# igashov/DiffLinker

Hardware: AMD Instinct MI355X
Metric: molecules/sec (500-step sample_chain) (higher is better)
Workload: dtype f32 (f16x3 split MFMA, fp32 accumulate)

## Files before the change

### difflinker_amd/csrc/egnn_fc.hip

```cpp
#include <hip/hip_runtime.h>
#include <stdint.h>
#include <stdlib.h>
#include <string.h>
#include <math.h>
#include <cmath>

#include <algorithm>
#include <atomic>
#include <vector>

#include "../../include/difflinker_hip.h"
#include "pack_layout.h"


namespace {

constexpr int LDH = 132;
constexpr int NMAX = 55;
constexpr int NQMAX = 2 * NMAX;
constexpr int THREADS = 512;
constexpr int NWAVES = THREADS / 64;
constexpr int GWAVES = 8;
constexpr int GTHREADS = 64 * GWAVES;
constexpr int L_A = 0;
// ... 18 lines not shown
constexpr int L_ZROW = L_XS + 4 * 56;
static_assert(L_ZROW + HID <= L_X0 && 56 >= NMAX + 1 && (L_ZROW % 4) == 0, "the zero row sits in the team-only part of the coordinate rows");
constexpr size_t LDS_BYTES = size_t(L_TOTAL) * 4;
static_assert(LDS_BYTES <= 163840, "LDS layout exceeds 160 KiB");
static_assert((L_B % 4) == 0 && (L_C % 4) == 0 && (L_W % 4) == 0 && (L_VEC % 4) == 0 && (L_XS % 4) == 0 &&
              (L_X0 % 4) == 0 && (L_Z % 4) == 0 && (L_DUMMY % 4) == 0, "16-byte alignment");
constexpr int L_TRIP3 = L_A + 2 * ST_CHUNK;
constexpr int L_AGGX3 = L_TRIP3 + 4 * 256;
static_assert(L_AGGX3 + 4 * (NMAX + 1) <= L_W && (L_TRIP3 % 4) == 0, "version-3 coordinate scratch must fit the h region behind the ring");

constexpr int TM_EPOCH = 2;
constexpr int TM_FAIL = 3;
constexpr int TM_ROWS = 4;
constexpr int TM_FLAGS = 6;
constexpr int TM_S = 8, TM_RANK = 9, TM_NOWN = 10;
constexpr int MS_NRCV = 12;
constexpr int MS_FULL = 13;
constexpr int CX_V3 = 38;

struct Lds {
    float *A, *B, *C, *W, *vec, *xs, *x0, *aggx, *z, *lm, *frag;
    int *idx, *rcv, *rpos, *misc;
    unsigned* fmax;
    float* dummy;
    int w;
};

__device__ __forceinline__ Lds lds_view(float* base) {
    Lds v;
    v.w = __builtin_amdgcn_readfirstlane(int(threadIdx.x) >> 6);
// ... 1232 lines not shown
    const float4* s4 = reinterpret_cast<const float4*>(wimg) + lane;
#pragma unroll
    for (int it = 0; it < ST_PIECES; ++it) {
        const int piece = HALF * 32 + it * 4 + hw;
        __builtin_amdgcn_global_load_lds((gptr_t)(s4 + piece * 64), (lptr_t)(v.W + piece * 256), 16, 0, 0);
    }
}
template <int N>
__device__ __forceinline__ void st_wait_vm() {
    if constexpr (N <= 0) asm volatile("s_waitcnt vmcnt(0)" ::: "memory");
    else asm volatile("s_waitcnt vmcnt(%0)" :: "n"(N) : "memory");
}
template <int V>
struct IC { static constexpr int value = V; };

template <bool TEAM, bool POST, bool NEXT_EQ>
__device__ __forceinline__ void stream_phase(const Lds& v, Prof& pf, const AggRegs* ar) {
    constexpr int NC = (POST ? 6 : 0) + 4;
    constexpr int C_P = POST ? 6 : 0;
    const PassCtx cx = pass_ctx(v);
    const LaneIds q = lane_ids(v);
    const int tid = q.tid, w = q.w, lane = q.lane;
    const int nb = cx.nb;
    const int nown = TEAM ? ctx_i(v, TM_NOWN) : nb;
    float* hs = cx.hs;
    const int pass_open = cx.pass + 1;
    const float* wp = ctx_p<const float>(v, CX_WP);
    const int sub = ctx_i(v, CX_SUB);
    const float* g = POST ? cx.g : nullptr;
    const float* nxb = pass_weights(wp, pass_open, sub);
    const NextPass nx = {nxb, NEXT_EQ};
    const float* sc = POST ? g + G_SCALE : nullptr;
    const float* scn = nxb + (NEXT_EQ ? E_SCALE : G_SCALE);
    const float* vecn = nxb + (NEXT_EQ ? E_VEC : G_VEC);
    float* lds0 = v.A - L_A;
    const bool loader = w >= ST_AWAVES;
    const int hw = w - ST_AWAVES, wa = w;
    const int n = lane & 15, kg = lane >> 4;
    const int ta = wa;
// ... 14 lines not shown
    float hmax = 0.f, aggmax = 0.f, s_agg = 1.f, s_t = 1.f, s_hn = 1.f, inv2 = 1.f;
    if constexpr (POST) {
        hmax = __uint_as_float(v.fmax[FM_H0 + par]);
        aggmax = __uint_as_float(v.fmax[FM_AGG]);
        s_agg = scale_for(aggmax);
        const float y3b = cload(sc, SC_L1_W3A) * hmax + cload(sc, SC_L1_W3B) * aggmax + cload(sc, SC_B3);
        s_t = scale_for(y3b);
        const float hnb = hmax + cload(sc, SC_L1_W4) * y3b + cload(sc, SC_B4);
        s_hn = scale_for(hnb);
        if (tid == 0 && (beyond_f16_range(aggmax) || beyond_f16_range(y3b) || beyond_f16_range(hnb))) atomicOr(&v.misc[1], NAN_RANGE | 3);
        inv2 = inv_pow2(s_t * cload(sc, 4));
    }
    const float s_h0 = scale_for(__uint_as_float(v.fmax[FM_H0 + par]));
    const float s_hf = POST ? s_hn : s_h0;
    constexpr int AGG_OFF = st_slot_off(st_slot(3, NC));
    if constexpr (POST) {
#pragma unroll
        for (int k = 0; k < 4; ++k) {
            const int e = tid + THREADS * k;
            if (e < nown * 32) *reinterpret_cast<float4*>(lds0 + AGG_OFF + (e >> 5) * LDH + 4 * (e & 31)) = ar->v[k];
        }
    }
    if (loader) {
        st_issue<st_slot(0, NC)>(lds0, chunk_src(0), hw, lane);
        prof_event(pf, w, lane, 200);
        auto lstep = [&](auto C_) {
            constexpr int C = decltype(C_)::value;
            constexpr int behind = (C >= 1 && C + 1 < NC ? ST_PIECES : 0) + (C == NC - 2 ? ST_PIECES : 0) + (C == NC - 1 ? 2 * ST_PIECES : 0);
            st_wait_vm<behind>();
            fine_event(pf, w, lane, 220 + C);
            lds_barrier();
// ... 10 lines not shown
        lstep(IC<0>{}); lstep(IC<1>{}); lstep(IC<2>{}); lstep(IC<3>{});
        if constexpr (NC > 4) { lstep(IC<4>{}); lstep(IC<5>{}); }
        if constexpr (NC > 6) { lstep(IC<6>{}); lstep(IC<7>{}); }
        if constexpr (NC > 8) { lstep(IC<8>{}); lstep(IC<9>{}); }
        fine_event(pf, w, lane, 240);
        lds_barrier();
        prof_event(pf, w, lane, 250);
    } else {
    BOp bh, bagg, bout, bin;
    floatx4 acc[4];
    float4 t0p[4];
    float4 res2[8], bb4[8];
    float4 Pout[8], Qout[8];
    float hm = 0.f;
    float S1 = 1.f;
    if (!TEAM) {
        const float x2 = __uint_as_float(v.fmax[FM_X2]), x02 = __uint_as_float(v.fmax[FM_X02]);
        S1 = fminf(scale_for(4.0f * x2) * scale_for(cload(scn, 6)), scale_for(4.0f * x02) * scale_for(cload(scn, 7)));
    }
    const float live = valid ? 1.0f : 0.0f;
    if (awave) {
        const float sb = s_h0 * live;
#pragma unroll
        for (int sl = 0; sl < 4; ++sl) {
            const float4 a = hold[2 * sl], c4 = hold[2 * sl + 1];
            const float u[8] = {a.x * sb, a.y * sb, a.z * sb, a.w * sb, c4.x * sb, c4.y * sb, c4.z * sb, c4.w * sb};
            split8t(u, bh.hi[sl], bh.lo[sl]);
        }
    }
    prof_event(pf, w, lane, 200);
    auto step = [&](auto C_) {
// ... 59 lines not shown
                const float4 a = res[2 * sp], c4 = res[2 * sp + 1];
                const float u[8] = {a.x, a.y, a.z, a.w, c4.x, c4.y, c4.z, c4.w};
                split8t(u, bout.hi[2 * half + sp], bout.lo[2 * half + sp]);
            }
            if constexpr (half == 1) bin = bout;
            if constexpr (C == 5) block_max(&v.fmax[FM_H0 + (par ^ 1)], hm, lane);
        }
    };
    step(IC<0>{}); step(IC<1>{}); step(IC<2>{}); step(IC<3>{});
    if constexpr (NC > 4) { step(IC<4>{}); step(IC<5>{}); }
    if constexpr (NC > 6) { step(IC<6>{}); step(IC<7>{}); }
    if constexpr (NC > 8) { step(IC<8>{}); step(IC<9>{}); }
    fine_event(pf, w, lane, 240);
    lds_barrier();
    prof_event(pf, w, lane, 250);
    if (valid) {
#pragma unroll
        for (int ot = 0; ot < 8; ++ot) {
            *reinterpret_cast<float4*>(v.A + l * LDH + 16 * ot + 4 * kg) = Pout[ot];
            *reinterpret_cast<float4*>(v.B + l * LDH + 16 * ot + 4 * kg) = Qout[ot];
        }
    }
    }
    if (tid == 0) {
        if constexpr (POST) { v.fmax[FS_HS] = __float_as_uint(s_hn); v.misc[CX_PAR] = par ^ 1; }
        v.misc[CX_PASS] = pass_open;
    }
    if constexpr (TEAM) {
        prof_event(pf, w, lane, 110);
        lds_barrier();
        team_exchange_q<1>(v, nb, tid, scn, pass_open == 0, POST ? (par ^ 1) : par, pf);
    }
    prof_event(pf, w, lane, 11);
    dma_wait();
    lds_barrier();
}


template <int PREC, bool TEAM, bool ATT>
__device__ __forceinline__ void gcl_pass3(const Lds& v, Prof& pf) {
    {
    const PassCtx cx = pass_ctx(v);
    const int nb = cx.nb, N = cx.N, par = cx.par;
    const int8_t* emask = cx.em;
    const float* sc = cx.g + G_SCALE;
    const LaneIds q = lane_ids(v);
    const int tid = q.tid, w = q.w, lane = q.lane;
    prof_event(pf, w, lane, 12);
    if (tid == 0) { v.fmax[FM_H0 + (par ^ 1)] = 0u; v.fmax[FM_AGG] = 0u; }
    const float hmax = __uint_as_float(v.fmax[TEAM ? FM_HG : FM_H0 + par]);
    const float x2 = __uint_as_float(v.fmax[FM_X2]), x02 = __uint_as_float(v.fmax[FM_X02]);
    const float pqb = (cload(sc, SC_L1_W1A) + cload(sc, SC_L1_W1B)) * hmax + cload(sc, SC_B1);
    const float u1b = pqb + 4.0f * (x2 * cload(sc, GS_WRW) + x02 * cload(sc, GS_WDW));
    const float sa = scale_for(u1b);
// ... 6 lines not shown
    }
    AggRegs ar;
    bool next_eq;
    {
        const PassCtx cx = pass_ctx(v);
        const int nown = TEAM ? ctx_i(v, TM_NOWN) : cx.nb;
        const LaneIds q = lane_ids(v);
        next_eq = cx.nx.equiv;
        lds_barrier();
        prof_event(pf, q.w, q.lane, 20);
        const float am = pair_reduce_gcl(v, nown, cx.nb, q.tid, ar, (cx.flags & 4) ? 1.0f / float(cx.N) : 1.0f);
        block_max(&v.fmax[FM_AGG], am, q.lane);
        prof_event(pf, q.w, q.lane, 21);
        lds_barrier();
        prof_event(pf, q.w, q.lane, 22);
    }
    if (next_eq) stream_phase<TEAM, true, true>(v, pf, &ar);
    else stream_phase<TEAM, true, false>(v, pf, &ar);
}

template <int PREC, bool TEAM>
__device__ __forceinline__ void equiv_pass3(const Lds& v, Prof& pf) {
    {
    const PassCtx cx = pass_ctx(v);
    const int nb = cx.nb, N = cx.N, par = cx.par;
    const int8_t* emask = cx.em;
    const float* sc = cx.g + E_SCALE;
    const float norm_constant = ctx_f(v, CX_NORMC);
    const LaneIds q = lane_ids(v);
    const int w = q.w, lane = q.lane;
    prof_event(pf, w, lane, 32);
    const float hmax = __uint_as_float(v.fmax[TEAM ? FM_HG : FM_H0 + par]);
    const float x2 = __uint_as_float(v.fmax[FM_X2]), x02 = __uint_as_float(v.fmax[FM_X02]);
    const float pqb = (cload(sc, SCE_L1_W5A) + cload(sc, SCE_L1_W5B)) * hmax + cload(sc, SCE_B5);
    const float u1b = pqb + 4.0f * (x2 * cload(sc, ES_WRW) + x02 * cload(sc, ES_WDW));
    const float sa = scale_for(u1b);
// ... 12 lines not shown
        }
    }
    pair_phase<true, PREC, false, TEAM>(v, nb, w, lane, emask, N, norm_constant, sa, inv_pow2(accs), sc,
                                        (cx.flags & 2) ? ctx_f(v, CX_CRANGE) : 0.0f, pf);
    prof_event(pf, w, lane, 33);
    }
    const PassCtx cx = pass_ctx(v);
    const int nb = cx.nb, N = cx.N;
    const int nown = TEAM ? ctx_i(v, TM_NOWN) : nb;
    const int S = TEAM ? ctx_i(v, TM_S) : 1, rank = TEAM ? ctx_i(v, TM_RANK) : 0;
    const bool more = cx.nx.base != nullptr;
    const LaneIds q = lane_ids(v);
    const int tid = q.tid, lane = q.lane;
    lds_barrier();
    const float xscale = (cx.flags & 4) ? 1.0f / float(N) : ((cx.flags & 2) ? ctx_f(v, CX_INVNORM) : 1.0f);
    pair_reduce_equiv<true>(v, nown, nb, tid, xscale);
    if (tid == 0) v.fmax[TEAM ? FM_XOWN : FM_X2] = 0u;
    lds_barrier();
    const float* aggx = v.A - L_A + L_AGGX3;
    float n2 = 0.0f;
    if (tid < nown) {
        const float lm = v.lm[tid];
        const int a = rank + tid * S;
        const bool moves = v.rpos[tid] >= 0;
#pragma unroll
        for (int k = 0; k < 3; ++k) {
            float xn = v.xs[4 * a + k];
            if (moves) {
                xn += aggx[4 * tid + k] * lm;
                v.xs[4 * a + k] = xn;
            }
            n2 = fmaf(xn, xn, n2);
        }
    }
    block_max(&v.fmax[TEAM ? FM_XOWN : FM_X2], n2, lane);
    prof_event(pf, q.w, lane, 34);
    lds_barrier();
    prof_event(pf, q.w, lane, 10);
    if (more) stream_phase<TEAM, false, false>(v, pf, nullptr);
}

template <bool TEAM>
__device__ __forceinline__ void head_phase(const Lds& v, bool v3);

template <int PREC, bool TEAM, bool ATT>
__device__ __forceinline__ void forward_molecule2(const Lds& v, Prof& pf) {
    const int tid = lane_ids(v).tid;
    const int nb = ctx_i(v, 0);
    const int nown = TEAM ? ctx_i(v, TM_NOWN) : nb;
    const int S = TEAM ? ctx_i(v, TM_S) : 1, rank = TEAM ? ctx_i(v, TM_RANK) : 0;
    const float* wp = ctx_p<const float>(v, CX_WP);
    float* hs = ctx_p<float>(v, CX_HS);
    const float tfeat = ctx_f(v, CX_TFEAT);
    const int nf = ctx_i(v, CX_NF), fin = ctx_i(v, CX_FIN);
    const int npass = ctx_i(v, CX_NPASS);
    const int w = __builtin_amdgcn_readfirstlane(tid >> 6);
    const int lane = tid & 63;
    const bool v3 = (PREC != 0) && !TEAM && nown > 32;
    if (tid == 0) { v.misc[CX_PASS] = v3 ? -1 : 0; v.misc[CX_PAR] = 0; v.misc[CX_V3] = v3 ? 1 : 0; }
    if (tid < 8) reinterpret_cast<int*>(v.A - L_A + L_PROG)[tid] = 0;
    if (!TEAM && tid < HID) (v.A - L_A + L_ZROW)[tid] = 0.0f;
    prof_event(pf, w, lane, 1);
    {
        if (tid < 8) v.fmax[tid] = 0u;
        __syncthreads();
    }
    const NextPass first = {wp + OFF_BLOCKS, false};
    if (!v3) stage_next(v, first, w, tid);
    if (tid < 4 * nown) {
        const int l = tid >> 2, k = tid & 3, a = rank + l * S;
        const float xv = (k < 3) ? v.z[l * DMAX + k] : 0.0f;
        v.xs[4 * a + k] = xv;
        v.x0[4 * a + k] = xv;
    }
    {
        float n2 = 0.0f;
        if (tid < nown) {
            const float x0 = v.z[tid * DMAX], x1 = v.z[tid * DMAX + 1], x2 = v.z[tid * DMAX + 2];
            n2 = x0 * x0 + x1 * x1 + x2 * x2;
        }
        const unsigned b = wave_max_u32(__float_as_uint(n2));
        if (lane == 0) {
            if (TEAM) lds_max_u32(&v.fmax[FM_XOWN], b);
            else { lds_max_u32(&v.fmax[FM_X2], b); lds_max_u32(&v.fmax[FM_X02], b); }
        }
    }
    {
        const int f = tid & (HID - 1);
        float wrow[FINP];
        const float4* wsrc = reinterpret_cast<const float4*>(wp + OFF_EMB_W + f * FINP);
#pragma unroll
        for (int q = 0; q < FINP / 4; ++q) {
            const float4 t4 = wsrc[q];
            wrow[4 * q] = t4.x; wrow[4 * q + 1] = t4.y; wrow[4 * q + 2] = t4.z; wrow[4 * q + 3] = t4.w;
        }
        const float be = wp[OFF_EMB_B + f];
        const float* ctxp = ctx_p<const float>(v, CX_CTXP);
        const int ct = ctx_i(v, CX_CT);
// ... 13 lines not shown
            if (v3) {
                hs[HS_HT + ((((l >> 4) * 8 + (f >> 4)) * 64 + 16 * ((f >> 2) & 3) + (l & 15)) * 4) + (f & 3)] = acc;
            } else {
            v.B[l * LDH + f] = acc;
            {
                const int r = l & 31;
                hs[HS_HT + ((((l >> 5) * 4 + (f >> 5)) * 4 + (r >> 3)) * 64 + (f & 31) + 32 * ((r >> 2) & 1)) * 4 + (r & 3)] = acc;
            }
            }
            hmax = fmaxf(hmax, fabsf(acc));
        }
        block_max(&v.fmax[FM_H0], hmax, lane);
    }
    __syncthreads();
    if (v3) {
        if constexpr (PREC != 0 && !TEAM) {
        if (tid == 0 && beyond_f16_range(__uint_as_float(v.fmax[FM_H0]))) atomicOr(&v.misc[1], NAN_RANGE | 3);
        prof_event(pf, w, lane, 2);
        stream_phase<TEAM, false, false>(v, pf, nullptr);
        const int sub = ctx_i(v, CX_SUB);
#pragma nounroll
        for (int p = 0; p < npass; p += sub + 1) {
#pragma nounroll
            for (int gi = 0; gi < sub; ++gi) gcl_pass3<PREC, TEAM, ATT>(v, pf);
            equiv_pass3<PREC, TEAM>(v, pf);
        }
        prof_event(pf, w, lane, 3);
        __syncthreads();
        head_phase<TEAM>(v, true);
        }
    } else {
    {
        const float s0 = (PREC != 0) ? scale_for(__uint_as_float(v.fmax[FM_H0])) : 1.0f;
        for (int e = tid; e < nown * 32; e += THREADS)
            put_quad<PREC>(v.C + (e >> 5) * LDH, 4 * (e & 31), *reinterpret_cast<const float4*>(v.B + (e >> 5) * LDH + 4 * (e & 31)), s0);
        if (PREC != 0 && tid == 0) {
            v.fmax[FS_HS] = __float_as_uint(s0);
            if (beyond_f16_range(__uint_as_float(v.fmax[FM_H0]))) atomicOr(&v.misc[1], NAN_RANGE | 3);
        }
    }
    __syncthreads();
    prof_event(pf, w, lane, 2);
    {
        PreW2 pw;
// ... 2 lines not shown
    }
    const int sub = ctx_i(v, CX_SUB);
#pragma nounroll
    for (int p = 0; p < npass; p += sub + 1) {
#pragma nounroll
        for (int gi = 0; gi < sub; ++gi) gcl_pass2<PREC, TEAM, ATT>(v, pf);
        equiv_pass2<PREC, TEAM>(v, pf);
    }
    prof_event(pf, w, lane, 3);
    __syncthreads();
    head_phase<TEAM>(v, false);
    }
    prof_event(pf, w, lane, 4);
}

template <bool TEAM>
__device__ __forceinline__ void head_phase(const Lds& v, bool v3) {
    const int tid = lane_ids(v).tid;
    const int nb = ctx_i(v, 0), nf = ctx_i(v, CX_NF);
    const int nown = TEAM ? ctx_i(v, TM_NOWN) : nb;
    const int S = TEAM ? ctx_i(v, TM_S) : 1, rank = TEAM ? ctx_i(v, TM_RANK) : 0;
    const float* wp = ctx_p<const float>(v, CX_WP);
    const float* hs = ctx_p<const float>(v, CX_HS);
    float* eps = v.A;
    int nanbits = 0;
    for (int e = tid; e < nown * nf; e += THREADS) {
        const int a = e / nf, o = e - a * nf;
        const int r = a & 31;
        const float* wo = wp + OFF_OUT_W + o * HID;
        float acc = wp[OFF_OUT_B + o];
        if (v3) {
            const float* hp = hs + HS_HT + ((a >> 4) * 8 * 64 + (a & 15)) * 4;
#pragma unroll
            for (int ot = 0; ot < 8; ++ot)
#pragma unroll
                for (int kg = 0; kg < 4; ++kg) {
// ... 17 lines not shown
        (void)r;
        eps[a * DMAX + 3 + o] = acc;
        if (acc != acc) nanbits |= 2;
    }
    if (tid < 4 * nown && (tid & 3) < 3) {
        const int l = tid >> 2, a = rank + l * S;
        const float vel = v.xs[4 * a + (tid & 3)] - v.x0[4 * a + (tid & 3)];
        eps[l * DMAX + (tid & 3)] = vel;
        if (vel != vel) nanbits |= 1;
    }
    if (TEAM && tid == 0 && v.misc[TM_FAIL] != 0) nanbits |= 8;
    if (nanbits) atomicOr(&v.misc[1], nanbits);
    __syncthreads();
}

__device__ __forceinline__ void build_receivers(const Lds& v, int nown, int tid) {
    if (tid < 64) {
        const bool rec = tid < nown && v.lm[tid] != 0.0f;
        const unsigned long long bal = __ballot(rec);
        const int pos = __popcll(bal & ((1ull << tid) - 1ull));
        if (rec) v.rcv[pos] = tid;
        if (tid < NMAX + 1) v.rpos[tid] = rec ? pos : -1;
        if (tid == 0) { v.misc[MS_NRCV] = __popcll(bal); v.misc[MS_FULL] = (__popcll(bal) == nown) ? 1 : 0; }
    }
}

__device__ __forceinline__ int compact_atoms(const Lds& v, const int8_t* __restrict__ node_mask_b, int N, int tid) {
    if (tid < 64) {
        int count = 0;
        for (int base = 0; base < N; base += 64) {
            const int a = base + tid;
            const bool real = (a < N) && (node_mask_b[a] != 0);
            const unsigned long long bal = __ballot(real);
// ... 28 lines not shown
    float* hsave;
};

struct TeamSlot {
    int slot, rank;
};
__device__ __forceinline__ TeamSlot team_slot(int k, int S) {
    const int group = k / (8 * S), within = k - group * 8 * S;
    TeamSlot t;
    t.slot = group * 8 + (within & 7);
    t.rank = within >> 3;
    return t;
}
__device__ __forceinline__ void team_init(const Lds& v, int nb, int S, int rank, char* rows, unsigned* flags, int fault) {
    const unsigned long long pr = reinterpret_cast<unsigned long long>(rows), pf = reinterpret_cast<unsigned long long>(flags);
    v.misc[TM_EPOCH] = 0; v.misc[TM_FAIL] = (fault != 0 && rank == 1) ? 1 : 0;
    v.misc[TM_ROWS] = int(unsigned(pr)); v.misc[TM_ROWS + 1] = int(unsigned(pr >> 32));
    v.misc[TM_FLAGS] = int(unsigned(pf)); v.misc[TM_FLAGS + 1] = int(unsigned(pf >> 32));
    v.misc[TM_S] = S; v.misc[TM_RANK] = rank;
    v.misc[TM_NOWN] = nb > rank ? (nb - rank + S - 1) / S : 0;
}

__device__ __forceinline__ void ctx_store(const Lds& v, const ModelDims& md, int N, const int8_t* em, float* hs, const float* wp,
                                          const float* ctx_rows, float tfeat, int mol) {
    v.misc[CX_N] = N;
    ctx_set_p(v, CX_EM, em); ctx_set_p(v, CX_HS, hs); ctx_set_p(v, CX_WP, wp); ctx_set_p(v, CX_CTXP, ctx_rows);
    v.misc[CX_PASS] = 0; v.misc[CX_PAR] = 0;
    v.misc[CX_FLAGS] = (md.attention ? 1 : 0) | (md.tanh ? 2 : 0) | (md.mean ? 4 : 0);
    v.misc[CX_NORMC] = __float_as_int(md.norm_constant); v.misc[CX_CRANGE] = __float_as_int(md.coords_range);
    v.misc[CX_INVNORM] = __float_as_int(md.inv_norm);
    v.misc[CX_NPASS] = (md.sub + 1) * md.n_layers; v.misc[CX_NF] = md.nf; v.misc[CX_FIN] = md.fin;
// ... 66 lines not shown
        }
    }
}

struct ChainArgs {
    const float* wpack;
    ModelDims md;
    dl_chain_args a;
    unsigned long long* prof;
    char* team_rows;
    unsigned* team_flags;
    int team_fault;
    float* hsave;
};

template <int PREC, bool TEAM, bool ATT>
__device__ __forceinline__ bool chain_step2(const Lds& v, int q) {
    {
        const auto* P = kargs<ChainArgs>();
        const int tid = lane_ids(v).tid;
        if (tid == 0) {
            const float t = (q == P->a.T) ? 0.0f : P->a.coefs[q].t;
            v.misc[CX_TFEAT] = __float_as_int(t);
        }
        __syncthreads();
    }
    Prof pf;
    pf.buf = (blockIdx.x == 0 && q == 0) ? kargs<ChainArgs>()->prof : nullptr;
    pf.n = 0;
    forward_molecule2<PREC, TEAM, ATT>(v, pf);
    const auto* P = kargs<ChainArgs>();
    const int tid = lane_ids(v).tid;
    const int b = ctx_i(v, CX_MOL), nb = ctx_i(v, 0);
    const int nown = TEAM ? ctx_i(v, TM_NOWN) : nb;
    const int S = TEAM ? ctx_i(v, TM_S) : 1, rank = TEAM ? ctx_i(v, TM_RANK) : 0;
    const int N = P->a.N, nf = P->md.nf, D = 3 + nf, T = P->a.T, K = P->a.keep_frames, B = P->a.B;
    if (v.misc[1] != 0) {
        if (!TEAM) {
            if (tid == 0) { P->a.nan_flags[b] = v.misc[1]; P->a.nan_step[b] = q; }
            return false;
        }
        if (tid == 0) {
            atomicOr(&P->a.nan_flags[b], v.misc[1]);
            atomicCAS(&P->a.nan_step[b], -1, q);
        }
    }
    const bool decode = (q == T);
    dl_step_coef cf;
    if (decode) { cf.t = 0.0f; cf.alpha_ts = 1.0f; cf.c_eps = 0.0f; cf.sigma = 0.0f; }
    else cf = P->a.coefs[q];
// ... 33 lines not shown
            }
        } else {
            const float mu = __fmul_rn(inv_alpha0, __fsub_rn(zt, __fmul_rn(sigma0, eh)));
            const float xh = __fadd_rn(mu, __fmul_rn(sigma_x, __fmul_rn(nz, lm)));
            const float zz = __fadd_rn(__fmul_rn(zt, fr), __fmul_rn(xh, lm));
            zn = (d < 3) ? __fmul_rn(zz, norm_x) : __fadd_rn(__fmul_rn(zz, norm_h), bias_h);
        }
        v.z[l * DMAX + d] = zn;
    }
    (void)fragm;
    if (TEAM && tid == 0) v.misc[1] = 0;
    __syncthreads();
    return true;
}

template <bool TEAM>
__device__ __forceinline__ bool chain_begin(const ChainArgs& p, const Lds& v, int b, int rank, int S, int qb, char* rows,
                                            unsigned* flags) {
    const dl_chain_args& g = p.a;
    const int tid = threadIdx.x;
    const int N = g.N, nf = p.md.nf, D = 3 + nf, K = g.keep_frames, B = g.B;
    const int limit = TEAM ? NQMAX : NMAX;
    if (g.skip_flags && g.skip_flags[b] != 0) return false;
    const int8_t* nm = g.node_mask + size_t(b) * N;
    const size_t frame = size_t(B) * N * D;
    float* chain_b = g.chain + size_t(b) * N * D;
    const int nb = compact_atoms(v, nm, N, tid);
    if (rank == 0) {
        if (tid == 0) {
            if (TEAM) { if (nb > limit) atomicOr(&g.nan_flags[b], 4); }
            else { g.nan_flags[b] = (nb > limit) ? 4 : 0; g.nan_step[b] = -1; }
        }
        for (int kf = 0; kf < K; ++kf)
            for (int e = tid; e < N * D; e += THREADS)
                if (nm[e / D] == 0 || nb > limit) chain_b[kf * frame + e] = 0.0f;
    }
    if (nb > limit || nb == 0) return false;
    if (tid == 0) {
        if (TEAM) team_init(v, nb, S, rank, rows, flags, p.team_fault);
        ctx_store(v, p.md, N, g.edge_mask ? g.edge_mask + size_t(b) * N * N : nullptr, p.hsave + size_t(blockIdx.x) * HS_STRIDE,
                  p.wpack, g.context ? g.context + size_t(b) * N * p.md.ctx : nullptr, 0.0f, b);
    }
    __syncthreads();
    const int nown = TEAM ? v.misc[TM_NOWN] : nb;
    if (tid < nown) {
        const size_t n = size_t(b) * N + v.idx[rank + tid * S];
        v.lm[tid] = g.linker_mask[n];
        v.frag[tid] = g.fragment_mask[n];
    }
    __syncthreads();
    build_receivers(v, nown, tid);
    const bool philox = (g.noise_x == nullptr);
    const unsigned gmol = unsigned(g.mol_offset + (g.mol_index ? g.mol_index[b] : b));
    for (int e = tid; e < nown * D; e += THREADS) {
        const int l = e / D, d = e - l * D;
        const int pos = v.idx[rank + l * S];
        const size_t n = size_t(b) * N + pos;
        float val, eps0;
        if (d < 3) { val = __fdiv_rn(g.x[n * 3 + d], g.norm_x); eps0 = philox ? 0.0f : g.noise_x[n * 3 + d]; }
        else { val = __fdiv_rn(__fsub_rn(g.h[n * nf + d - 3], g.bias_h), g.norm_h); eps0 = philox ? 0.0f : g.noise_h[n * nf + d - 3]; }
        if (philox) eps0 = philox_normal(g.noise_seed, gmol, unsigned(pos), 0u, unsigned(d));
        const float lm = v.lm[l];
        float z0 = __fadd_rn(__fmul_rn(val, v.frag[l]), __fmul_rn(__fmul_rn(eps0, lm), lm));
        if (qb > 0) z0 = g.z_state[n * D + d];
        v.z[l * DMAX + d] = z0;
    }
    __syncthreads();
    return true;
}

template <bool TEAM>
__device__ __forceinline__ void chain_end(const Lds& v, int qe, int T) {
    if (qe <= T) {
        const auto* P = kargs<ChainArgs>();
        const int tid = lane_ids(v).tid;
        const int b = ctx_i(v, CX_MOL), nb = ctx_i(v, 0), D = 3 + P->md.nf, N = P->a.N;
        const int nown = TEAM ? ctx_i(v, TM_NOWN) : nb;
        const int S = TEAM ? ctx_i(v, TM_S) : 1, rank = TEAM ? ctx_i(v, TM_RANK) : 0;
        for (int e = tid; e < nown * D; e += THREADS) {
            const int l = e / D, d = e - l * D;
            P->a.z_state[(size_t(b) * N + v.idx[rank + l * S]) * D + d] = v.z[l * DMAX + d];
        }
        return;
    }
    {
        const auto* P = kargs<ChainArgs>();
        const int tid = lane_ids(v).tid;
        const int b = ctx_i(v, CX_MOL), nb = ctx_i(v, 0), nf = P->md.nf, D = 3 + nf;
        const int nown = TEAM ? ctx_i(v, TM_NOWN) : nb;
        const int S = TEAM ? ctx_i(v, TM_S) : 1, rank = TEAM ? ctx_i(v, TM_RANK) : 0;
        if (tid < nown) {
            const int l = tid;
            float* o = P->a.chain + size_t(b) * P->a.N * D + v.idx[rank + l * S] * D;
            o[0] = v.z[l * DMAX + 0]; o[1] = v.z[l * DMAX + 1]; o[2] = v.z[l * DMAX + 2];
            int best = 0;
            float bv = v.z[l * DMAX + 3];
            for (int kk = 1; kk < nf; ++kk) {
                const float hv = v.z[l * DMAX + 3 + kk];
                if (hv > bv) { bv = hv; best = kk; }
            }
            for (int kk = 0; kk < nf; ++kk) o[3 + kk] = (kk == best) ? 1.0f : 0.0f;
        }
        if (TEAM && tid == 0 && v.misc[TM_FAIL] != 0) atomicOr(&P->a.nan_flags[b], 8);
    }
}
// ... 82 lines not shown
    }
    if (alive) chain_end<false>(v, qe, T);
    const int j = p.team_of[b];
    if (j < 0) return;
    const int rank = qe <= T ? 0 : 1;
    const int bo = rank == 0 ? b : p.team_mol[j];
    const unsigned mine = rank == 1 ? JW_HERE : alive ? JW_READY : JW_DEAD;
    const unsigned other = join_meet(v, p.words + size_t(j) * JOIN_WORDS, rank, mine,
                                     p.wait_ticks ? p.wait_ticks + size_t(j) * 2 : nullptr);
    if (mine == JW_DEAD || other == JW_DEAD) return;
    if (other == JW_POISON) {
        if (threadIdx.x == 0) atomicOr(&p.c.a.nan_flags[bo], 8);
        return;
    }
    const int qb = p.c.a.q_end[bo];
    if (!chain_begin<true>(p.c, v, bo, rank, 2, qb, p.c.team_rows + size_t(j) * TEAM_MOL_BYTES,
                           p.c.team_flags + size_t(j) * TEAM_MAX)) return;
#pragma nounroll
    for (int q = qb; q <= T; ++q) chain_step2<PREC, true, ATT>(v, q);
    chain_end<true>(v, T + 1, T);
}

__global__ void sampler_step_kernel(int total, int D, const float* __restrict__ z_t, const float* __restrict__ eps_hat,
                                    const float* __restrict__ noise, const float* __restrict__ frag,
                                    const float* __restrict__ lmask, dl_step_coef cf, float* __restrict__ z_s) {
    const int e = blockIdx.x * blockDim.x + threadIdx.x;
    if (e >= total) return;
    const int n = e / D;
    const float lm = lmask[n];
    const float zt = z_t[e];
    const float eh = __fmul_rn(eps_hat[e], lm);
    const float mu = __fsub_rn(__fdiv_rn(zt, cf.alpha_ts), __fmul_rn(cf.c_eps, eh));
    const float zs = __fadd_rn(mu, __fmul_rn(cf.sigma, __fmul_rn(noise[e], lm)));
    z_s[e] = __fadd_rn(__fmul_rn(zt, frag[n]), __fmul_rn(zs, lm));
}

thread_local int g_last_hip = 0;
#ifdef DL_TEST_HOOKS
std::atomic<int> g_team_fault{0};
#endif
unsigned long long* g_prof_buf = nullptr;

inline int take_team_fault() {
#ifdef DL_TEST_HOOKS
    int n = g_team_fault.load();
    while (n > 0 && !g_team_fault.compare_exchange_weak(n, n - 1)) {}
    return n > 0 ? 1 : 0;
#else
    return 0;
#endif
}

inline bool hip_ok(hipError_t e) {
    if (e != hipSuccess) { g_last_hip = int(e); return false; }
    return true;
}

void pack_unit(float* dst, const float* w, int ld, int col0, double scale) {
    for (int nt = 0; nt < 4; ++nt)
        for (int sg = 0; sg < 16; ++sg)
            for (int lane = 0; lane < 64; ++lane)
                for (int j = 0; j < 4; ++j) {
// ... 239 lines not shown

}

extern "C" {

int32_t dl_abi_version(void) { return DL_ABI_VERSION; }
#ifdef DL_PROFILE
int32_t dl_profile_max_events(void) { return PROF_MAX_EVENTS; }
#else
int32_t dl_profile_max_events(void) { return 0; }
#endif
void dl_set_profile_buffer(void* device_buf) { g_prof_buf = static_cast<unsigned long long*>(device_buf); }
int32_t dl_last_hip_error(void) { return g_last_hip; }
int32_t dl_max_atoms(void) { return NMAX; }
#ifdef DL_TEST_HOOKS
void dl_debug_team_fault(int32_t launches) { g_team_fault.store(launches < 0 ? 0 : launches); }
#endif

const char* dl_error_string(int32_t s) {
    switch (s) {
        case DL_OK: return "ok";
        case DL_ERR_BAD_ARG: return "bad argument";
        case DL_ERR_UNSUPPORTED: return "hyper-parameter not supported by the HIP path";
        case DL_ERR_TOO_MANY_ATOMS: return "molecule exceeds dl_max_atoms()";
        case DL_ERR_HIP: return "HIP runtime error";
        case DL_ERR_NO_DEVICE: return "no HIP device";
        case DL_ERR_ALLOC: return "allocation failed";
        default: return "unknown";
    }
}

// ... 551 lines not shown
```

Measured before the change: 573.7.

## Add owner-computes split for two-block team molecules

For two-block teams handling molecules with 33–55 atoms, one block (the owner) now runs the full streaming forward over all atoms. The helper block does only the pairwise aggregation passes for half the receivers and publishes its results through the team exchange buffer. This replaces the symmetric split, where both blocks ran the stream phase and exchanged q rows, and is meant to cut duplicated work and exchange traffic. The cost is extra cross-block syncs each pass, load imbalance between owner and helper, and a large amount of new synchronisation code. Test fault-injection hooks are also extended so either rank can be made to fail.

```diff
diff --git a/difflinker_amd/csrc/egnn_fc.hip b/difflinker_amd/csrc/egnn_fc.hip
--- a/difflinker_amd/csrc/egnn_fc.hip
+++ b/difflinker_amd/csrc/egnn_fc.hip
@@ -56,6 +56,7 @@
 constexpr int TM_ROWS = 4;
 constexpr int TM_FLAGS = 6;
 constexpr int TM_S = 8, TM_RANK = 9, TM_NOWN = 10;
+constexpr int TM_OC = 11;
 constexpr int MS_NRCV = 12;
 constexpr int MS_FULL = 13;
 constexpr int CX_V3 = 38;
@@ -1318,15 +1319,143 @@
 template <int V>
 struct IC { static constexpr int value = V; };
 
-template <bool TEAM, bool POST, bool NEXT_EQ>
+constexpr int OC_AGG_OFF = st_slot_off(st_slot(3, 10));
+constexpr int OC_NOWN0 = (NMAX + 1) / 2;
+static_assert(OC_NOWN0 + NMAX / 2 <= NMAX + 1 && NMAX + OC_NOWN0 <= NQMAX, "owner-computes: rows of the triples and of the exchange");
+struct OcX {
+    __amdgpu_buffer_rsrc_t rows;
+    int pbase, hbase;
+    unsigned epoch;
+};
+__device__ __forceinline__ OcX oc_x(const Lds& v) {
+    OcX x;
+    x.epoch = unsigned(v.misc[TM_EPOCH]);
+    x.rows = team_rows(v);
+    x.pbase = int(x.epoch & 1u) * (NQMAX * TX_ROW * 4);
+    x.hbase = TEAM_X_BYTES + int(x.epoch & 1u) * (TEAM_MAX * 16);
+    return x;
+}
+__device__ __forceinline__ u32x4 oc_bits(const float4& f) {
+    return u32x4{__float_as_uint(f.x), __float_as_uint(f.y), __float_as_uint(f.z), __float_as_uint(f.w)};
+}
+__device__ __forceinline__ float4 oc_floats(const u32x4& b) {
+    return make_float4(__uint_as_float(b.x), __uint_as_float(b.y), __uint_as_float(b.z), __uint_as_float(b.w));
+}
+__device__ __forceinline__ void oc_publish_a(const Lds& v, int nb, int tid, int par) {
+    const OcX x = oc_x(v);
+    for (int e = tid; e < nb * 33; e += THREADS) {
+        const int l = e / 33, q4 = e - l * 33;
+        const float4 val = (q4 < 32) ? *reinterpret_cast<const float4*>(v.B + l * LDH + 4 * q4)
+                                     : *reinterpret_cast<const float4*>(v.xs + 4 * l);
+        __builtin_amdgcn_raw_buffer_store_b128(oc_bits(val), x.rows, x.pbase + (l * TX_ROW + 4 * q4) * 4, 0, 16);
+    }
+    if (tid == 0) {
+        const unsigned hb = v.fmax[FM_H0 + par];
+        const u32x4 hdr = {hb, v.fmax[FM_X2], 0u, 0u};
+        __builtin_amdgcn_raw_buffer_store_b128(hdr, x.rows, x.hbase, 0, 16);
+        v.fmax[FM_HG] = hb;
+    }
+    team_sync(v, tid, x.epoch);
+}
+__device__ __forceinline__ void oc_fetch_a(const Lds& v, int nb, int tid) {
+    const int nown = v.misc[TM_NOWN];
+    const bool first = v.misc[CX_PASS] == 0;
+    const OcX x = oc_x(v);
+    team_sync(v, tid, x.epoch);
+    const u32x4 hdr = __builtin_amdgcn_raw_buffer_load_b128(x.rows, x.hbase, 0, 16);
+    const u32x4 xb = __builtin_amdgcn_raw_buffer_load_b128(x.rows, x.pbase + (min(tid, nb - 1) * TX_ROW + HID) * 4, 0, 16);
+    u32x4 qv[4], pv[2];
+#pragma unroll
+    for (int k = 0; k < 4; ++k) {
+        const int e = min(tid + THREADS * k, nb * 32 - 1);
+        qv[k] = __builtin_amdgcn_raw_buffer_load_b128(x.rows, x.pbase + ((e >> 5) * TX_ROW + 4 * (e & 31)) * 4, 0, 16);
+    }
+#pragma unroll
+    for (int k = 0; k < 2; ++k) {
+        const int e = max(min(tid + THREADS * k, nown * 32 - 1), 0);
+        pv[k] = __builtin_amdgcn_raw_buffer_load_b128(x.rows, x.pbase + ((NMAX + (e >> 5)) * TX_ROW + 4 * (e & 31)) * 4, 0, 16);
+    }
+    if (tid < nb) {
+        const float4 xv = make_float4(__uint_as_float(xb.x), __uint_as_float(xb.y), __uint_as_float(xb.z), 0.0f);
+        *reinterpret_cast<float4*>(v.xs + 4 * tid) = xv;
+        if (first) *reinterpret_cast<float4*>(v.x0 + 4 * tid) = xv;
+    }
+    if (tid == 0) {
+        v.fmax[FM_HG] = hdr.x; v.fmax[FM_X2] = hdr.y;
+        if (first) v.fmax[FM_X02] = hdr.y;
+    }
+#pragma unroll
+    for (int k = 0; k < 4; ++k) {
+        const int e = tid + THREADS * k;
+        if (e < nb * 32) *reinterpret_cast<float4*>(v.B + (e >> 5) * LDH + 4 * (e & 31)) = oc_floats(qv[k]);
+    }
+#pragma unroll
+    for (int k = 0; k < 2; ++k) {
+        const int e = tid + THREADS * k;
+        if (e < nown * 32) *reinterpret_cast<float4*>(v.A + (e >> 5) * LDH + 4 * (e & 31)) = oc_floats(pv[k]);
+    }
+}
+__device__ __forceinline__ void oc_publish_b_gcl(const Lds& v, int nown, int tid, const AggRegs& ar) {
+    const OcX x = oc_x(v);
+#pragma unroll
+    for (int k = 0; k < 4; ++k) {
+        const int e = tid + THREADS * k;
+        if (e < nown * 32)
+            __builtin_amdgcn_raw_buffer_store_b128(oc_bits(ar.v[k]), x.rows, x.pbase + ((NMAX + (e >> 5)) * TX_ROW + 4 * (e & 31)) * 4, 0, 16);
+    }
+    if (tid == 0) {
+        const u32x4 hdr = {v.fmax[FM_AGG], 0u, 0u, 0u};
+        __builtin_amdgcn_raw_buffer_store_b128(hdr, x.rows, x.hbase + 16, 0, 16);
+    }
+    team_sync(v, tid, x.epoch);
+}
+__device__ __forceinline__ void oc_fetch_b_gcl(const Lds& v, int nb, int tid) {
+    const int nh = nb >> 1;
+    const OcX x = oc_x(v);
+    team_sync(v, tid, x.epoch);
+    const u32x4 hdr = __builtin_amdgcn_raw_buffer_load_b128(x.rows, x.hbase + 16, 0, 16);
+    u32x4 av[2];
+#pragma unroll
+    for (int k = 0; k < 2; ++k) {
+        const int e = min(tid + THREADS * k, nh * 32 - 1);
+        av[k] = __builtin_amdgcn_raw_buffer_load_b128(x.rows, x.pbase + ((NMAX + (e >> 5)) * TX_ROW + 4 * (e & 31)) * 4, 0, 16);
+    }
+    if (tid == 0) v.fmax[FM_AGG] = max(v.fmax[FM_AGG], hdr.x);
+    float* aggrows = v.A - L_A + OC_AGG_OFF;
+#pragma unroll
+    for (int k = 0; k < 2; ++k) {
+        const int e = tid + THREADS * k;
+        if (e < nh * 32) *reinterpret_cast<float4*>(aggrows + (1 + 2 * (e >> 5)) * LDH + 4 * (e & 31)) = oc_floats(av[k]);
+    }
+}
+__device__ __forceinline__ void oc_publish_b_equiv(const Lds& v, int nown, int tid) {
+    const OcX x = oc_x(v);
+    if (tid < nown) {
+        const bool moves = v.rpos[tid] >= 0;
+        const float4 t = *reinterpret_cast<const float4*>(v.aggx + 4 * tid);
+        const float4 val = moves ? make_float4(t.x, t.y, t.z, 1.0f) : make_float4(0.f, 0.f, 0.f, 0.f);
+        __builtin_amdgcn_raw_buffer_store_b128(oc_bits(val), x.rows, x.pbase + (NMAX + tid) * TX_ROW * 4, 0, 16);
+    }
+    team_sync(v, tid, x.epoch);
+}
+__device__ __forceinline__ void oc_fetch_b_equiv(const Lds& v, int nb, int tid) {
+    const int nh = nb >> 1;
+    const OcX x = oc_x(v);
+    team_sync(v, tid, x.epoch);
+    const u32x4 t = __builtin_amdgcn_raw_buffer_load_b128(x.rows, x.pbase + (NMAX + min(tid, nh - 1)) * TX_ROW * 4, 0, 16);
+    if (tid < nh) *reinterpret_cast<float4*>(v.A - L_A + L_AGGX3 + 4 * (OC_NOWN0 + tid)) = oc_floats(t);
+}
+
+template <bool TEAM, bool POST, bool NEXT_EQ, int OC = 0>
 __device__ __forceinline__ void stream_phase(const Lds& v, Prof& pf, const AggRegs* ar) {
+    static_assert(OC == 0 || (OC == 1 && TEAM), "owner-computes: the owner's phase");
     constexpr int NC = (POST ? 6 : 0) + 4;
     constexpr int C_P = POST ? 6 : 0;
     const PassCtx cx = pass_ctx(v);
     const LaneIds q = lane_ids(v);
     const int tid = q.tid, w = q.w, lane = q.lane;
     const int nb = cx.nb;
-    const int nown = TEAM ? ctx_i(v, TM_NOWN) : nb;
+    const int nown = (TEAM && OC == 0) ? ctx_i(v, TM_NOWN) : nb;
     float* hs = cx.hs;
     const int pass_open = cx.pass + 1;
     const float* wp = ctx_p<const float>(v, CX_WP);
@@ -1371,7 +1500,15 @@
     const float s_h0 = scale_for(__uint_as_float(v.fmax[FM_H0 + par]));
     const float s_hf = POST ? s_hn : s_h0;
     constexpr int AGG_OFF = st_slot_off(st_slot(3, NC));
-    if constexpr (POST) {
+    if constexpr (POST && OC != 0) {
+        static_assert(AGG_OFF == OC_AGG_OFF, "oc_fetch_b_gcl writes the helper's rows here");
+        const int nrec = ctx_i(v, TM_NOWN);
+#pragma unroll
+        for (int k = 0; k < 4; ++k) {
+            const int e = tid + THREADS * k;
+            if (e < nrec * 32) *reinterpret_cast<float4*>(lds0 + AGG_OFF + 2 * (e >> 5) * LDH + 4 * (e & 31)) = ar->v[k];
+        }
+    } else if constexpr (POST) {
 #pragma unroll
         for (int k = 0; k < 4; ++k) {
             const int e = tid + THREADS * k;
@@ -1412,7 +1549,7 @@
     float4 Pout[8], Qout[8];
     float hm = 0.f;
     float S1 = 1.f;
-    if (!TEAM) {
+    if (!TEAM || OC != 0) {
         const float x2 = __uint_as_float(v.fmax[FM_X2]), x02 = __uint_as_float(v.fmax[FM_X02]);
         S1 = fminf(scale_for(4.0f * x2) * scale_for(cload(scn, 6)), scale_for(4.0f * x02) * scale_for(cload(scn, 7)));
     }
@@ -1502,6 +1639,17 @@
     fine_event(pf, w, lane, 240);
     lds_barrier();
     prof_event(pf, w, lane, 250);
+    if constexpr (OC != 0) {
+        const OcX x = oc_x(v);
+        if (valid) {
+#pragma unroll
+            for (int ot = 0; ot < 8; ++ot) {
+                *reinterpret_cast<float4*>(v.B + l * LDH + 16 * ot + 4 * kg) = Qout[ot];
+                if ((l & 1) == 0) *reinterpret_cast<float4*>(v.A + (l >> 1) * LDH + 16 * ot + 4 * kg) = Pout[ot];
+                else __builtin_amdgcn_raw_buffer_store_b128(oc_bits(Pout[ot]), x.rows, x.pbase + ((NMAX + (l >> 1)) * TX_ROW + 16 * ot + 4 * kg) * 4, 0, 16);
+            }
+        }
+    } else
     if (valid) {
 #pragma unroll
         for (int ot = 0; ot < 8; ++ot) {
@@ -1514,7 +1662,11 @@
         if constexpr (POST) { v.fmax[FS_HS] = __float_as_uint(s_hn); v.misc[CX_PAR] = par ^ 1; }
         v.misc[CX_PASS] = pass_open;
     }
-    if constexpr (TEAM) {
+    if constexpr (OC != 0) {
+        prof_event(pf, w, lane, 110);
+        lds_barrier();
+        oc_publish_a(v, nb, tid, POST ? (par ^ 1) : par);
+    } else if constexpr (TEAM) {
         prof_event(pf, w, lane, 110);
         lds_barrier();
         team_exchange_q<1>(v, nb, tid, scn, pass_open == 0, POST ? (par ^ 1) : par, pf);
@@ -1525,7 +1677,7 @@
 }
 
 
-template <int PREC, bool TEAM, bool ATT>
+template <int PREC, bool TEAM, bool ATT, int OC = 0>
 __device__ __forceinline__ void gcl_pass3(const Lds& v, Prof& pf) {
     {
     const PassCtx cx = pass_ctx(v);
@@ -1562,12 +1714,24 @@
         prof_event(pf, q.w, q.lane, 21);
         lds_barrier();
         prof_event(pf, q.w, q.lane, 22);
-    }
-    if (next_eq) stream_phase<TEAM, true, true>(v, pf, &ar);
-    else stream_phase<TEAM, true, false>(v, pf, &ar);
-}
-
-template <int PREC, bool TEAM>
+        if constexpr (OC == 2) {
+            stage_next(v, cx.nx, q.w, q.tid);
+            if (q.tid == 0) v.misc[CX_PASS] = cx.pass + 1;
+            oc_publish_b_gcl(v, nown, q.tid, ar);
+            return;
+        }
+        if constexpr (OC == 1) {
+            oc_fetch_b_gcl(v, cx.nb, q.tid);
+            lds_barrier();
+        }
+    }
+    if constexpr (OC != 2) {
+        if (next_eq) stream_phase<TEAM, true, true, OC>(v, pf, &ar);
+        else stream_phase<TEAM, true, false, OC>(v, pf, &ar);
+    }
+}
+
+template <int PREC, bool TEAM, int OC = 0>
 __device__ __forceinline__ void equiv_pass3(const Lds& v, Prof& pf) {
     {
     const PassCtx cx = pass_ctx(v);
@@ -1610,6 +1774,45 @@
     const int tid = q.tid, lane = q.lane;
     lds_barrier();
     const float xscale = (cx.flags & 4) ? 1.0f / float(N) : ((cx.flags & 2) ? ctx_f(v, CX_INVNORM) : 1.0f);
+    if constexpr (OC == 2) {
+        pair_reduce_equiv<false>(v, nown, nb, tid, xscale);
+        lds_barrier();
+        stage_next(v, cx.nx, q.w, tid);
+        if (tid == 0) v.misc[CX_PASS] = cx.pass + 1;
+        oc_publish_b_equiv(v, nown, tid);
+        return;
+    }
+    if constexpr (OC == 1) {
+        pair_reduce_equiv<true>(v, nown, nb, tid, xscale);
+        if (tid == 0) v.fmax[FM_X2] = 0u;
+        oc_fetch_b_equiv(v, nb, tid);
+        lds_barrier();
+        const float* aggx = v.A - L_A + L_AGGX3;
+        float n2 = 0.0f;
+        if (tid < nb) {
+            const float lm = v.lm[tid];
+            const int li = tid >> 1;
+            const float4 t = *reinterpret_cast<const float4*>(aggx + 4 * ((tid & 1) ? OC_NOWN0 + li : li));
+            const bool moves = (tid & 1) ? (t.w != 0.0f) : (v.rpos[li] >= 0);
+            const float tk[3] = {t.x, t.y, t.z};
+#pragma unroll
+            for (int k = 0; k < 3; ++k) {
+                float xn = v.xs[4 * tid + k];
+                if (moves) {
+                    xn += tk[k] * lm;
+                    v.xs[4 * tid + k] = xn;
+                }
+                n2 = fmaf(xn, xn, n2);
+            }
+        }
+        block_max(&v.fmax[FM_X2], n2, lane);
+        prof_event(pf, q.w, lane, 34);
+        lds_barrier();
+        prof_event(pf, q.w, lane, 10);
+        if (more) stream_phase<TEAM, false, false, 1>(v, pf, nullptr);
+        return;
+    }
+    if constexpr (OC == 0) {
     pair_reduce_equiv<true>(v, nown, nb, tid, xscale);
     if (tid == 0) v.fmax[TEAM ? FM_XOWN : FM_X2] = 0u;
     lds_barrier();
@@ -1634,17 +1837,19 @@
     lds_barrier();
     prof_event(pf, q.w, lane, 10);
     if (more) stream_phase<TEAM, false, false>(v, pf, nullptr);
-}
-
-template <bool TEAM>
+    }
+}
+
+template <bool TEAM, int OC = 0>
 __device__ __forceinline__ void head_phase(const Lds& v, bool v3);
 
-template <int PREC, bool TEAM, bool ATT>
+template <int PREC, bool TEAM, bool ATT, int OC = 0>
 __device__ __forceinline__ void forward_molecule2(const Lds& v, Prof& pf) {
+    static_assert(OC == 0 || (OC == 1 && TEAM && PREC != 0 && !ATT), "owner-computes: the owner's forward");
     const int tid = lane_ids(v).tid;
     const int nb = ctx_i(v, 0);
-    const int nown = TEAM ? ctx_i(v, TM_NOWN) : nb;
-    const int S = TEAM ? ctx_i(v, TM_S) : 1, rank = TEAM ? ctx_i(v, TM_RANK) : 0;
+    const int nown = (TEAM && OC == 0) ? ctx_i(v, TM_NOWN) : nb;
+    const int S = (TEAM && OC == 0) ? ctx_i(v, TM_S) : 1, rank = (TEAM && OC == 0) ? ctx_i(v, TM_RANK) : 0;
     const float* wp = ctx_p<const float>(v, CX_WP);
     float* hs = ctx_p<float>(v, CX_HS);
     const float tfeat = ctx_f(v, CX_TFEAT);
@@ -1652,7 +1857,7 @@
     const int npass = ctx_i(v, CX_NPASS);
     const int w = __builtin_amdgcn_readfirstlane(tid >> 6);
     const int lane = tid & 63;
-    const bool v3 = (PREC != 0) && !TEAM && nown > 32;
+    const bool v3 = OC != 0 || ((PREC != 0) && !TEAM && nown > 32);
     if (tid == 0) { v.misc[CX_PASS] = v3 ? -1 : 0; v.misc[CX_PAR] = 0; v.misc[CX_V3] = v3 ? 1 : 0; }
     if (tid < 8) reinterpret_cast<int*>(v.A - L_A + L_PROG)[tid] = 0;
     if (!TEAM && tid < HID) (v.A - L_A + L_ZROW)[tid] = 0.0f;
@@ -1677,7 +1882,7 @@
         }
         const unsigned b = wave_max_u32(__float_as_uint(n2));
         if (lane == 0) {
-            if (TEAM) lds_max_u32(&v.fmax[FM_XOWN], b);
+            if (TEAM && OC == 0) lds_max_u32(&v.fmax[FM_XOWN], b);
             else { lds_max_u32(&v.fmax[FM_X2], b); lds_max_u32(&v.fmax[FM_X02], b); }
         }
     }
@@ -1721,20 +1926,20 @@
     }
     __syncthreads();
     if (v3) {
-        if constexpr (PREC != 0 && !TEAM) {
+        if constexpr (PREC != 0 && (!TEAM || OC != 0)) {
         if (tid == 0 && beyond_f16_range(__uint_as_float(v.fmax[FM_H0]))) atomicOr(&v.misc[1], NAN_RANGE | 3);
         prof_event(pf, w, lane, 2);
-        stream_phase<TEAM, false, false>(v, pf, nullptr);
+        stream_phase<TEAM, false, false, OC>(v, pf, nullptr);
         const int sub = ctx_i(v, CX_SUB);
 #pragma nounroll
         for (int p = 0; p < npass; p += sub + 1) {
 #pragma nounroll
-            for (int gi = 0; gi < sub; ++gi) gcl_pass3<PREC, TEAM, ATT>(v, pf);
-            equiv_pass3<PREC, TEAM>(v, pf);
+            for (int gi = 0; gi < sub; ++gi) gcl_pass3<PREC, TEAM, ATT, OC>(v, pf);
+            equiv_pass3<PREC, TEAM, OC>(v, pf);
         }
         prof_event(pf, w, lane, 3);
         __syncthreads();
-        head_phase<TEAM>(v, true);
+        head_phase<TEAM, OC>(v, true);
         }
     } else {
     {
@@ -1767,12 +1972,41 @@
     prof_event(pf, w, lane, 4);
 }
 
-template <bool TEAM>
+template <int PREC>
+__device__ __forceinline__ void forward_oc_helper(const Lds& v, Prof& pf) {
+    const LaneIds q0 = lane_ids(v);
+    const int tid = q0.tid;
+    const int npass = ctx_i(v, CX_NPASS), sub = ctx_i(v, CX_SUB);
+    if (tid == 0) { v.misc[CX_PASS] = 0; v.misc[CX_PAR] = 0; v.misc[CX_V3] = 0; }
+    if (tid < 8) { reinterpret_cast<int*>(v.A - L_A + L_PROG)[tid] = 0; v.fmax[tid] = 0u; }
+    __syncthreads();
+    {
+        const NextPass first = {ctx_p<const float>(v, CX_WP) + OFF_BLOCKS, false};
+        stage_next(v, first, q0.w, tid);
+    }
+    auto open = [&]() {
+        oc_fetch_a(v, ctx_i(v, 0), lane_ids(v).tid);
+        dma_wait();
+        lds_barrier();
+    };
+#pragma nounroll
+    for (int p = 0; p < npass; p += sub + 1) {
+#pragma nounroll
+        for (int gi = 0; gi < sub; ++gi) {
+            open();
+            gcl_pass3<PREC, true, false, 2>(v, pf);
+        }
+        open();
+        equiv_pass3<PREC, true, 2>(v, pf);
+    }
+}
+
+template <bool TEAM, int OC>
 __device__ __forceinline__ void head_phase(const Lds& v, bool v3) {
     const int tid = lane_ids(v).tid;
     const int nb = ctx_i(v, 0), nf = ctx_i(v, CX_NF);
-    const int nown = TEAM ? ctx_i(v, TM_NOWN) : nb;
-    const int S = TEAM ? ctx_i(v, TM_S) : 1, rank = TEAM ? ctx_i(v, TM_RANK) : 0;
+    const int nown = (TEAM && OC == 0) ? ctx_i(v, TM_NOWN) : nb;
+    const int S = (TEAM && OC == 0) ? ctx_i(v, TM_S) : 1, rank = (TEAM && OC == 0) ? ctx_i(v, TM_RANK) : 0;
     const float* wp = ctx_p<const float>(v, CX_WP);
     const float* hs = ctx_p<const float>(v, CX_HS);
     float* eps = v.A;
@@ -1820,9 +2054,9 @@
     __syncthreads();
 }
 
-__device__ __forceinline__ void build_receivers(const Lds& v, int nown, int tid) {
+__device__ __forceinline__ void build_receivers(const Lds& v, int nown, int tid, int stride = 1) {
     if (tid < 64) {
-        const bool rec = tid < nown && v.lm[tid] != 0.0f;
+        const bool rec = tid < nown && v.lm[stride * tid] != 0.0f;
         const unsigned long long bal = __ballot(rec);
         const int pos = __popcll(bal & ((1ull << tid) - 1ull));
         if (rec) v.rcv[pos] = tid;
@@ -1881,7 +2115,7 @@
 }
 __device__ __forceinline__ void team_init(const Lds& v, int nb, int S, int rank, char* rows, unsigned* flags, int fault) {
     const unsigned long long pr = reinterpret_cast<unsigned long long>(rows), pf = reinterpret_cast<unsigned long long>(flags);
-    v.misc[TM_EPOCH] = 0; v.misc[TM_FAIL] = (fault != 0 && rank == 1) ? 1 : 0;
+    v.misc[TM_EPOCH] = 0; v.misc[TM_FAIL] = (fault != 0 && rank == 2 - fault) ? 1 : 0;
     v.misc[TM_ROWS] = int(unsigned(pr)); v.misc[TM_ROWS + 1] = int(unsigned(pr >> 32));
     v.misc[TM_FLAGS] = int(unsigned(pf)); v.misc[TM_FLAGS + 1] = int(unsigned(pf >> 32));
     v.misc[TM_S] = S; v.misc[TM_RANK] = rank;
@@ -1978,7 +2212,7 @@
     float* hsave;
 };
 
-template <int PREC, bool TEAM, bool ATT>
+template <int PREC, bool TEAM, bool ATT, int OC = 0>
 __device__ __forceinline__ bool chain_step2(const Lds& v, int q) {
     {
         const auto* P = kargs<ChainArgs>();
@@ -1992,12 +2226,18 @@
     Prof pf;
     pf.buf = (blockIdx.x == 0 && q == 0) ? kargs<ChainArgs>()->prof : nullptr;
     pf.n = 0;
-    forward_molecule2<PREC, TEAM, ATT>(v, pf);
+    if constexpr (OC == 2) {
+        forward_oc_helper<PREC>(v, pf);
+        if (lane_ids(v).tid == 0) v.misc[1] = 0;
+        __syncthreads();
+        return true;
+    }
+    forward_molecule2<PREC, TEAM, ATT, (OC == 1 ? 1 : 0)>(v, pf);
     const auto* P = kargs<ChainArgs>();
     const int tid = lane_ids(v).tid;
     const int b = ctx_i(v, CX_MOL), nb = ctx_i(v, 0);
-    const int nown = TEAM ? ctx_i(v, TM_NOWN) : nb;
-    const int S = TEAM ? ctx_i(v, TM_S) : 1, rank = TEAM ? ctx_i(v, TM_RANK) : 0;
+    const int nown = (TEAM && OC == 0) ? ctx_i(v, TM_NOWN) : nb;
+    const int S = (TEAM && OC == 0) ? ctx_i(v, TM_S) : 1, rank = (TEAM && OC == 0) ? ctx_i(v, TM_RANK) : 0;
     const int N = P->a.N, nf = P->md.nf, D = 3 + nf, T = P->a.T, K = P->a.keep_frames, B = P->a.B;
     if (v.misc[1] != 0) {
         if (!TEAM) {
@@ -2061,9 +2301,11 @@
     return true;
 }
 
-template <bool TEAM>
-__device__ __forceinline__ bool chain_begin(const ChainArgs& p, const Lds& v, int b, int rank, int S, int qb, char* rows,
+template <bool TEAM, bool OCJ = false>
+__device__ __forceinline__ bool chain_begin(const ChainArgs& p, const Lds& v, int b, int rank_, int S_, int qb, char* rows,
                                             unsigned* flags) {
+    const int rank_pair = rank_, S_pair = S_;
+    int rank = rank_, S = S_;
     const dl_chain_args& g = p.a;
     const int tid = threadIdx.x;
     const int N = g.N, nf = p.md.nf, D = 3 + nf, K = g.keep_frames, B = g.B;
@@ -2084,19 +2326,26 @@
     }
     if (nb > limit || nb == 0) return false;
     if (tid == 0) {
-        if (TEAM) team_init(v, nb, S, rank, rows, flags, p.team_fault);
+        if (TEAM) team_init(v, nb, S_pair, rank_pair, rows, flags, p.team_fault);
         ctx_store(v, p.md, N, g.edge_mask ? g.edge_mask + size_t(b) * N * N : nullptr, p.hsave + size_t(blockIdx.x) * HS_STRIDE,
                   p.wpack, g.context ? g.context + size_t(b) * N * p.md.ctx : nullptr, 0.0f, b);
+        if (OCJ) v.misc[TM_OC] = (S_pair == 2 && nb > 32 && nb <= NMAX) ? 1 + rank_pair : 0;
     }
     __syncthreads();
-    const int nown = TEAM ? v.misc[TM_NOWN] : nb;
+    int nown = TEAM ? v.misc[TM_NOWN] : nb;
+    bool oc_owner = false;
+    if constexpr (OCJ) {
+        oc_owner = v.misc[TM_OC] == 1;
+        if (oc_owner) { nown = nb; rank = 0; S = 1; }
+    }
     if (tid < nown) {
         const size_t n = size_t(b) * N + v.idx[rank + tid * S];
         v.lm[tid] = g.linker_mask[n];
         v.frag[tid] = g.fragment_mask[n];
     }
     __syncthreads();
-    build_receivers(v, nown, tid);
+    if (OCJ && oc_owner) build_receivers(v, v.misc[TM_NOWN], tid, 2);
+    else build_receivers(v, nown, tid);
     const bool philox = (g.noise_x == nullptr);
     const unsigned gmol = unsigned(g.mol_offset + (g.mol_index ? g.mol_index[b] : b));
     for (int e = tid; e < nown * D; e += THREADS) {
@@ -2116,14 +2365,14 @@
     return true;
 }
 
-template <bool TEAM>
+template <bool TEAM, int OC = 0>
 __device__ __forceinline__ void chain_end(const Lds& v, int qe, int T) {
     if (qe <= T) {
         const auto* P = kargs<ChainArgs>();
         const int tid = lane_ids(v).tid;
         const int b = ctx_i(v, CX_MOL), nb = ctx_i(v, 0), D = 3 + P->md.nf, N = P->a.N;
-        const int nown = TEAM ? ctx_i(v, TM_NOWN) : nb;
-        const int S = TEAM ? ctx_i(v, TM_S) : 1, rank = TEAM ? ctx_i(v, TM_RANK) : 0;
+        const int nown = OC == 2 ? 0 : (TEAM && OC == 0) ? ctx_i(v, TM_NOWN) : nb;
+        const int S = (TEAM && OC == 0) ? ctx_i(v, TM_S) : 1, rank = (TEAM && OC == 0) ? ctx_i(v, TM_RANK) : 0;
         for (int e = tid; e < nown * D; e += THREADS) {
             const int l = e / D, d = e - l * D;
             P->a.z_state[(size_t(b) * N + v.idx[rank + l * S]) * D + d] = v.z[l * DMAX + d];
@@ -2134,8 +2383,8 @@
         const auto* P = kargs<ChainArgs>();
         const int tid = lane_ids(v).tid;
         const int b = ctx_i(v, CX_MOL), nb = ctx_i(v, 0), nf = P->md.nf, D = 3 + nf;
-        const int nown = TEAM ? ctx_i(v, TM_NOWN) : nb;
-        const int S = TEAM ? ctx_i(v, TM_S) : 1, rank = TEAM ? ctx_i(v, TM_RANK) : 0;
+        const int nown = OC == 2 ? 0 : (TEAM && OC == 0) ? ctx_i(v, TM_NOWN) : nb;
+        const int S = (TEAM && OC == 0) ? ctx_i(v, TM_S) : 1, rank = (TEAM && OC == 0) ? ctx_i(v, TM_RANK) : 0;
         if (tid < nown) {
             const int l = tid;
             float* o = P->a.chain + size_t(b) * P->a.N * D + v.idx[rank + l * S] * D;
@@ -2248,8 +2497,24 @@
         return;
     }
     const int qb = p.c.a.q_end[bo];
-    if (!chain_begin<true>(p.c, v, bo, rank, 2, qb, p.c.team_rows + size_t(j) * TEAM_MOL_BYTES,
-                           p.c.team_flags + size_t(j) * TEAM_MAX)) return;
+    constexpr bool OCJ = PREC != 0 && !ATT;
+    if (!chain_begin<true, OCJ>(p.c, v, bo, rank, 2, qb, p.c.team_rows + size_t(j) * TEAM_MOL_BYTES,
+                                p.c.team_flags + size_t(j) * TEAM_MAX)) return;
+    if constexpr (OCJ) {
+        const int oc = ctx_i(v, TM_OC);
+        if (oc == 1) {
+#pragma nounroll
+            for (int q = qb; q <= T; ++q) chain_step2<PREC, true, ATT, 1>(v, q);
+            chain_end<true, 1>(v, T + 1, T);
+            return;
+        }
+        if (oc == 2) {
+#pragma nounroll
+            for (int q = qb; q <= T; ++q) chain_step2<PREC, true, ATT, 2>(v, q);
+            chain_end<true, 2>(v, T + 1, T);
+            return;
+        }
+    }
 #pragma nounroll
     for (int q = qb; q <= T; ++q) chain_step2<PREC, true, ATT>(v, q);
     chain_end<true>(v, T + 1, T);
@@ -2278,8 +2543,8 @@
 inline int take_team_fault() {
 #ifdef DL_TEST_HOOKS
     int n = g_team_fault.load();
-    while (n > 0 && !g_team_fault.compare_exchange_weak(n, n - 1)) {}
-    return n > 0 ? 1 : 0;
+    while (n != 0 && !g_team_fault.compare_exchange_weak(n, n > 0 ? n - 1 : n + 1)) {}
+    return n > 0 ? 1 : n < 0 ? 2 : 0;
 #else
     return 0;
 #endif
@@ -2549,7 +2814,7 @@
 int32_t dl_last_hip_error(void) { return g_last_hip; }
 int32_t dl_max_atoms(void) { return NMAX; }
 #ifdef DL_TEST_HOOKS
-void dl_debug_team_fault(int32_t launches) { g_team_fault.store(launches < 0 ? 0 : launches); }
+void dl_debug_team_fault(int32_t launches) { g_team_fault.store(launches); }
 #endif
 
 const char* dl_error_string(int32_t s) {
```

After: 558.5. 0.974x the previous value.
